# xiaozhah/Aligner

Hardware: AMD Instinct MI355X
Metric: aligned utterances/sec + frames/sec, [B=64,T_text=200,T_mel=1000] (higher is better)
Workload: dtype f32; 1 GPU; configs[1]: similarity (L2, C=80) + monotonic alignment search, [B=64,T_text=200,T_mel=1000] fp32 per GPU, dense fp32 path + int32 durations out; batch_per_gpu=64, t_text=200, t_mel=1000, c_att=80, launch=hipGraph, batches_in_flight=3, parallelism=batch-sharded x1

## Files before the change

aligner_amd/csrc/api.cpp:

```cpp
#include <cstdarg>
#include <cstdio>
#include <cstdlib>

#include <mutex>
#include <cstring>
#include <map>
#include <utility>

#include "common.h"

namespace aligner {

char *error_buffer() {
    static thread_local char buf[512] = {0};
    return buf;
}

unsigned long long *g_debug_stamps = nullptr;

static int env_flag(const char *name) { const char *e = getenv(name); return e && e[0] && e[0] != '0'; }
int g_opt_fwdsum_one_wave = env_flag("ALIGNER_FWDSUM_ONE_WAVE");
int g_opt_fwdsum_serial = env_flag("ALIGNER_FWDSUM_SERIAL");
int g_opt_fwdsum_no_grad_stager = 0;
int g_opt_softattn_exact = env_flag("ALIGNER_SOFTATTN_EXACT");
int g_opt_mobo_drop_segment = -1;
int g_opt_mobo_start_lag = 0;
int g_opt_mobo_lanes = 0;
int g_opt_mobo_bwd_general = 0;
int g_opt_softattn_no_pair = 0;
int g_opt_softattn_rt_drop_merge = 0;
int g_opt_softattn_strips = env_flag("ALIGNER_SOFTATTN_STRIPS");
int g_opt_softattn_split = 0;
int g_opt_conv_narrow_ft = 0;
int g_opt_conv_no_ring = 0;
int g_opt_conv_no_fuse = 0;
int g_opt_conv_split_always = env_flag("ALIGNER_CONV_SPLIT_ALWAYS");
int g_opt_maxpath_no_split_walk = 0;
int g_opt_maxpath_zero_blocks = 0;
int g_opt_maxpath_no_mask_verify = 0;
int g_opt_maxpath_no_optimistic_mask = 0;
int g_opt_mobo_full_chain = 0;
int g_opt_mobo_stamp_wave = 0;

hipError_t ensure_dynamic_lds(const void *kernel, size_t bytes) {
    if (bytes <= 64 * 1024) return hipSuccess;
    int dev = 0;
    hipError_t e = hipGetDevice(&dev);
    if (e != hipSuccess) return e;
    static std::mutex mu;
    static std::map<std::pair<int, const void *>, size_t> granted;
    std::lock_guard<std::mutex> lock(mu);
    const auto key = std::make_pair(dev, kernel);
    auto it = granted.find(key);
    if (it != granted.end() && it->second >= bytes) return hipSuccess;
    e = hipFuncSetAttribute(kernel, hipFuncAttributeMaxDynamicSharedMemorySize, (int)bytes);
    if (e == hipSuccess) granted[key] = bytes;
    return e;
}

int device_cu_count() {
    int dev = 0, v = 0;
    if (hipGetDevice(&dev) != hipSuccess) return 1;
    static std::mutex mu;
    static std::map<int, int> counts;
    std::lock_guard<std::mutex> lock(mu);
    auto it = counts.find(dev);
    if (it != counts.end()) return it->second;
    if (hipDeviceGetAttribute(&v, hipDeviceAttributeMultiprocessorCount, dev) != hipSuccess || v < 1) v = 1;
    counts[dev] = v;
    return v;
}

int device_lds_limit() {
    int dev = 0;
    if (hipGetDevice(&dev) != hipSuccess) return 64 * 1024;
    static std::mutex mu;
    static std::map<int, int> limits;
    std::lock_guard<std::mutex> lock(mu);
    auto it = limits.find(dev);
    if (it != limits.end()) return it->second;
    int lim = 64 * 1024, v = 0;
    hipDeviceProp_t prop;
    if (hipGetDeviceProperties(&prop, dev) == hipSuccess && std::strncmp(prop.gcnArchName, "gfx950", 6) == 0)
        lim = 160 * 1024;
    else if (hipDeviceGetAttribute(&v, hipDeviceAttributeMaxSharedMemoryPerBlock, dev) == hipSuccess && v > 0)
        lim = v;
    limits[dev] = lim;
    return lim;
}

int fail(int code, const char *fmt, ...) {
    va_list ap;
    va_start(ap, fmt);
    vsnprintf(error_buffer(), 512, fmt, ap);
    va_end(ap);
    return code;
}

}

extern "C" {

int aligner_abi_version(void) { return ALIGNER_ABI_VERSION; }

const char *aligner_last_error(void) { return aligner::error_buffer(); }

void aligner_debug_set_stamps(void *stamps_dev) {
    aligner::g_debug_stamps = static_cast<unsigned long long *>(stamps_dev);
}

int aligner_debug_set_option(const char *name, int value) {
    if (!name) return aligner::fail(ALIGNER_EINVAL, "null option name");
    if (std::strcmp(name, "fwdsum_one_wave") == 0) { aligner::g_opt_fwdsum_one_wave = value; return ALIGNER_OK; }
    if (std::strcmp(name, "fwdsum_no_grad_stager") == 0) { aligner::g_opt_fwdsum_no_grad_stager = value; return ALIGNER_OK; }
    if (std::strcmp(name, "fwdsum_serial") == 0) { aligner::g_opt_fwdsum_serial = value; return ALIGNER_OK; }
    if (std::strcmp(name, "softattn_exact") == 0) { aligner::g_opt_softattn_exact = value; return ALIGNER_OK; }
    if (std::strcmp(name, "mobo_start_lag") == 0) { aligner::g_opt_mobo_start_lag = value; return ALIGNER_OK; }
    if (std::strcmp(name, "mobo_lanes") == 0) { aligner::g_opt_mobo_lanes = value; return ALIGNER_OK; }
    if (std::strcmp(name, "mobo_stamp_wave") == 0) { aligner::g_opt_mobo_stamp_wave = value; return ALIGNER_OK; }
    if (std::strcmp(name, "mobo_full_chain") == 0) { aligner::g_opt_mobo_full_chain = value; return ALIGNER_OK; }
    if (std::strcmp(name, "softattn_split") == 0) { aligner::g_opt_softattn_split = value; return ALIGNER_OK; }
    if (std::strcmp(name, "conv_narrow_ft") == 0) { aligner::g_opt_conv_narrow_ft = value; return ALIGNER_OK; }
    if (std::strcmp(name, "conv_no_ring") == 0) { aligner::g_opt_conv_no_ring = value; return ALIGNER_OK; }
    if (std::strcmp(name, "conv_no_fuse") == 0) { aligner::g_opt_conv_no_fuse = value; return ALIGNER_OK; }
    if (std::strcmp(name, "conv_split_always") == 0) { aligner::g_opt_conv_split_always = value; return ALIGNER_OK; }
    if (std::strcmp(name, "maxpath_no_optimistic_mask") == 0) { aligner::g_opt_maxpath_no_optimistic_mask = value; return ALIGNER_OK; }
    if (std::strcmp(name, "maxpath_no_mask_verify") == 0) { aligner::g_opt_maxpath_no_mask_verify = value; return ALIGNER_OK; }
    if (std::strcmp(name, "maxpath_zero_blocks") == 0) { aligner::g_opt_maxpath_zero_blocks = value; return ALIGNER_OK; }
    if (std::strcmp(name, "maxpath_no_split_walk") == 0) { aligner::g_opt_maxpath_no_split_walk = value; return ALIGNER_OK; }
    if (std::strcmp(name, "softattn_strips") == 0) { aligner::g_opt_softattn_strips = value; return ALIGNER_OK; }
    if (std::strcmp(name, "softattn_rt_drop_merge") == 0) { aligner::g_opt_softattn_rt_drop_merge = value; return ALIGNER_OK; }
    if (std::strcmp(name, "softattn_no_pair") == 0) { aligner::g_opt_softattn_no_pair = value; return ALIGNER_OK; }
    if (std::strcmp(name, "mobo_bwd_general") == 0) { aligner::g_opt_mobo_bwd_general = value; return ALIGNER_OK; }
    if (std::strcmp(name, "mobo_drop_segment") == 0) { aligner::g_opt_mobo_drop_segment = value; return ALIGNER_OK; }
    return aligner::fail(ALIGNER_EINVAL, "unknown option '%s'", name);
}

int aligner_device_count(void) {
    int n = 0;
    if (hipGetDeviceCount(&n) != hipSuccess) {
        (void)hipGetLastError();
        return 0;
    }
    return n;
}

}
```

aligner_amd/csrc/common.h:

```cpp
#pragma once
#include <hip/hip_runtime.h>
#include <cstdarg>
#include <cstdio>

#include "aligner_amd.h"

namespace aligner {

char *error_buffer();
int   fail(int code, const char *fmt, ...) __attribute__((format(printf, 2, 3)));

#define ALIGNER_HIP_CHECK(expr)                                                        \
    do {                                                                               \
        hipError_t _e = (expr);                                                        \
        if (_e != hipSuccess)                                                          \
            return ::aligner::fail(ALIGNER_EHIP, "%s failed: %s (%s:%d)", #expr,       \
                                   hipGetErrorString(_e), __FILE__, __LINE__);         \
    } while (0)

inline int dtype_size(int dt) {
    switch (dt) {
        case ALIGNER_DT_F32: return 4;
        case ALIGNER_DT_F16: return 2;
        case ALIGNER_DT_BF16: return 2;
        case ALIGNER_DT_F64: return 8;
        case ALIGNER_DT_I32: return 4;
        case ALIGNER_DT_U8: return 1;
        case ALIGNER_DT_I64: return 8;
        default: return 0;
    }
}

hipError_t ensure_dynamic_lds(const void *kernel, size_t bytes);

int device_lds_limit();
int device_cu_count();

extern unsigned long long *g_debug_stamps;
extern int g_opt_softattn_exact;
extern int g_opt_mobo_start_lag;
extern int g_opt_mobo_stamp_wave;
extern int g_opt_mobo_full_chain;
extern int g_opt_conv_narrow_ft;
extern int g_opt_conv_no_ring;
extern int g_opt_maxpath_no_optimistic_mask;
extern int g_opt_maxpath_no_mask_verify;
extern int g_opt_maxpath_zero_blocks;
extern int g_opt_maxpath_no_split_walk;
extern int g_opt_conv_no_fuse;
extern int g_opt_conv_split_always;
extern int g_opt_softattn_split;
extern int g_opt_softattn_strips;
extern int g_opt_softattn_rt_drop_merge;
extern int g_opt_softattn_no_pair;
extern int g_opt_mobo_bwd_general;
extern int g_opt_mobo_lanes;
extern int g_opt_mobo_drop_segment;
extern int g_opt_fwdsum_no_grad_stager;
extern int g_opt_fwdsum_serial;
extern int g_opt_fwdsum_one_wave;

inline size_t align_up(size_t v, size_t a) { return (v + a - 1) / a * a; }

}
```

aligner_amd/csrc/mobo.hip:

```cpp
#include <hip/hip_runtime.h>

#include <cmath>
#include <cstdint>

#include "aligner_amd.h"
#include "common.h"

namespace aligner {

constexpr float MB_NEG = -1e30f;
constexpr float MB_DEADF = -1e7f;
constexpr int MB_DEADM = -(1 << 24);
constexpr unsigned MB_FILL = 0xFFFFFFFFu;
constexpr float MB_LOG2E = 1.4426950408889634f, MB_LN2 = 0.6931471805599453f;
constexpr int MB_SPIN_LIMIT = 1 << 21;

struct MoboParams {
    const void *e;
    const int *t_xs, *t_ys;
    float *log_alpha;
    int *boundaries;
    int *durations;
    float *map_score;
    float *Lw;
// ... 225 lines not shown
    __syncthreads();
    const int Rb = s_blockmax;
    bool fits = true;
    for (int x = tid; x < NE; x += 256) {
        const int M = sM[x];
        sT[x] = __builtin_ldexpf(sS[x], M - Rb);
        if (M != MB_DEADM && M < Rb - 100) fits = false;
    }
    const int slow = __syncthreads_or(!fits);
    const int xb = 4 * tid;
    float Ls[4] = {MB_NEG, MB_NEG, MB_NEG, MB_NEG};
    if (k0 + xb < p.Ty) {
        if (!slow && D >= 8) {
            const float *t = sT + xb;
            const float4 h = *reinterpret_cast<const float4 *>(t);
            float core = h.w;
            int c = 4;
            for (; c + 8 <= D; c += 8) {
                const float4 a = *reinterpret_cast<const float4 *>(t + c), bq = *reinterpret_cast<const float4 *>(t + c + 4);
                core += ((a.x + a.y) + (a.z + a.w)) + ((bq.x + bq.y) + (bq.z + bq.w));
            }
            for (; c < D; ++c) core += t[c];
            const float e0 = t[D], e1 = t[D + 1], e2 = t[D + 2];
            const float acc[4] = {core + ((h.x + h.y) + h.z), core + ((h.y + h.z) + e0), core + ((h.z + e0) + e1),
                                  core + ((e0 + e1) + e2)};
#pragma unroll
            for (int u = 0; u < 4; ++u)
                if (acc[u] > 0.f) Ls[u] = (float)Rb + __builtin_amdgcn_logf(acc[u]);
        } else if (!slow) {
#pragma unroll 1
            for (int u = 0; u < 4; ++u) {
                float acc = 0.f;
                for (int c = 0; c < D; ++c) acc += sT[xb + u + c];
                if (acc > 0.f) Ls[u] = (float)Rb + __builtin_amdgcn_logf(acc);
            }
        } else {
#pragma unroll 1
            for (int u = 0; u < 4; ++u) {
                int Mw, qb;
                float acc, best;
                mb_window<false>(sM + xb + u, sS + xb + u, nullptr, D, Mw, acc, best, qb);
                if (acc > 0.f) Ls[u] = (float)Mw + __builtin_amdgcn_logf(acc);
            }
        }
#pragma unroll
        for (int u = 0; u < 4; ++u) {
            const int k = k0 + xb + u;
            if (k < p.Ty) {
                p.Lw[rowoff + k] = (k < J && k >= klo && k <= khi) ? Ls[u] : MB_NEG;
                if (p.log_alpha && k >= J) p.log_alpha[rowoff + k] = -__builtin_huge_valf();
            }
        }
    }
}

__device__ __forceinline__ void mb_ring_store(unsigned *p, unsigned v) {
    __hip_atomic_store(p, v, __ATOMIC_RELAXED, __HIP_MEMORY_SCOPE_AGENT);
}
__device__ __forceinline__ unsigned mb_ring_load(const unsigned *p) {
    return __hip_atomic_load(p, __ATOMIC_RELAXED, __HIP_MEMORY_SCOPE_AGENT);
}

struct MbSeg {
    int a, bnd, D, J, W;
    bool has_next;
    int *sM;
    float *sS, *sV;
    unsigned *ring_out;
};
__device__ __forceinline__ void mb_phase1(const MbSeg &g, int i, int bo, int k, float la, float de, float Lraw) {
    const float L = (k < g.J) ? Lraw : MB_NEG;
    const bool live = L > MB_DEADF;
    const float u = (live && la > MB_DEADF) ? la - L : MB_NEG;
    float v = (live && de > MB_DEADF) ? de - L : MB_NEG;
    v = (v > MB_DEADF) ? v : MB_NEG;
    int M;
    float s;
    mb_encode(u, M, s);
    const int x = bo + g.D + (k - g.a);
    g.sM[x] = M;
    g.sS[x] = s;
    g.sV[x] = v;
    if (g.has_next && k >= g.bnd - g.D) {
        unsigned *r = g.ring_out + (size_t)i * 3 * g.D + (k - (g.bnd - g.D));
        mb_ring_store(r, __builtin_bit_cast(unsigned, (float)M));
        mb_ring_store(r + g.D, __builtin_bit_cast(unsigned, s));
        mb_ring_store(r + 2 * g.D, __builtin_bit_cast(unsigned, v));
    }
}
__device__ __forceinline__ void mb_phase2(const MbSeg &g, int bo, int j, int lo, int hi, float ev, float &lav, float &dev,
                                          int &dur) {
    lav = MB_NEG;
    dev = MB_NEG;
    dur = 0;
    if (j >= lo && j <= hi) {
        int Mw, qb;
        float acc, best;
        const int x = bo + (j - g.a);
        mb_window<true>(g.sM + x, g.sS + x, g.sV + x, g.D, Mw, acc, best, qb);
        if (acc > 0.f && ev > MB_DEADF) lav = ev + ((float)Mw + __builtin_amdgcn_logf(acc));
        if (best > MB_DEADF && ev > MB_DEADF) {
            dev = ev + best;
            dur = g.D - qb;
        }
        lav = (lav > MB_DEADF) ? lav : MB_NEG;
        dev = (dev > MB_DEADF) ? dev : MB_NEG;
// ... 967 lines not shown
                for (const int r8 = cnt & 7; c < r8; ++c) acc += t[c];
                for (; c < cnt; c += 8)
                    acc += ((t[c] + t[c + 1]) + (t[c + 2] + t[c + 3])) + ((t[c + 4] + t[c + 5]) + (t[c + 6] + t[c + 7]));
#pragma unroll
                for (int m = 1; m < H; m <<= 1) acc += mb_quad_xor_f(acc, m);
                if (acc > 0.f) lsum = (float)R + __builtin_amdgcn_logf(acc);
            } else {
                int Mw, qb;
                float acc, best;
                mb_window<false>(sM + x, sS + x, nullptr, cnt, Mw, acc, best, qb);
#pragma unroll
                for (int m = 1; m < H; m <<= 1) {
                    const int Mo = mb_quad_xor_i(Mw, m);
                    const float ao = mb_quad_xor_f(acc, m);
                    const int Mn = Mw > Mo ? Mw : Mo;
                    acc = __builtin_ldexpf(acc, Mw - Mn) + __builtin_ldexpf(ao, Mo - Mn);
                    Mw = Mn;
                }
                if (acc > 0.f) lsum = (float)Mw + __builtin_amdgcn_logf(acc);
            }
            float lav = MB_NEG;
            if (feasible && ev > MB_DEADF && lsum > MB_DEADF) lav = ev + lsum;
            lav = (lav > MB_DEADF) ? lav : MB_NEG;
            la = lav;
            R = (Rn != MB_DEADM) ? Rn : R;
            float *lp = (lead && j1 >= 1) ? p.log_alpha + ro + (j1 - 1) : reinterpret_cast<float *>(trash);
            *lp = (lav > MB_DEADF) ? lav * MB_LN2 : -__builtin_huge_valf();
        }
    };
#pragma unroll 1
    for (int i = i0; i <= i1; i += 2) {
        do_row(i, e_n1, L_n1);
        if (i + 1 > i1) break;
        do_row(i + 1, e_n2, L_n2);
    }
    if (i1 + 1 < I) {
        const int i = i1 + 1;
        if (publishes) {
            const float Lr = p.Lw[ubase + (size_t)i * p.Ty + kl];
            const float L = (j1 < J) ? Lr : MB_NEG;
            const float u = (L > MB_DEADF && la > MB_DEADF) ? la - L : MB_NEG;
            int M;
            float sm;
            mb_encode(u, M, sm);
            unsigned *r = ring_out + (size_t)i * 3 * D + (j1 - (bnd - D));
            mb_ring_store(r, __builtin_bit_cast(unsigned, (float)M));
            mb_ring_store(r + D, __builtin_bit_cast(unsigned, sm));
        }
        if (lead && j1 >= 1) p.log_alpha[ubase + (size_t)i * p.Ty + (j1 - 1)] = -__builtin_huge_valf();
        dead_rows(i1 + 2, I);
    }
}

__global__ __launch_bounds__(256) void mobo_backtrack_kernel(MoboParams p, int RB) {
    extern __shared__ __attribute__((aligned(16))) unsigned char smem[];
    __shared__ int s_j, s_bad;
    __shared__ int s_b[64], s_d[64];
    typedef unsigned piece_t __attribute__((ext_vector_type(4)));
    piece_t *win = reinterpret_cast<piece_t *>(smem);
    const int tid = threadIdx.x, b = blockIdx.x, D = p.D;
    int I = p.t_xs[b], J = p.t_ys[b];
    I = I > p.Tx ? p.Tx : I;
    J = J > p.Ty ? p.Ty : J;
    const bool ok = I >= 1 && J >= I && (long long)J <= (long long)I * D;
    int *bo = p.boundaries + (size_t)b * p.Tx;
    int *du = p.durations ? p.durations + (size_t)b * p.Tx : nullptr;
    if (!ok || p.failw[b]) {
        for (int i = tid; i < p.Tx; i += 256) {
            bo[i] = 0;
            if (du) du[i] = 0;
        }
        if (p.map_score && tid == 0) p.map_score[b] = -__builtin_huge_valf();
        return;
    }
    for (int i = I + tid; i < p.Tx; i += 256) {
        bo[i] = J;
        if (du) du[i] = 0;
    }
    const unsigned short *backb = p.back + (size_t)b * p.Tx * p.bstride;
    const int tpr = 256 / RB, t_of = tid / tpr, c_of = tid - t_of * tpr;
    const int wp = ((RB - 1) * D + 8) / 8 + 1;
    if (tid == 0) { s_j = J; s_bad = 0; }
    __syncthreads();
    for (int i = I - 1; i >= 0; i -= RB) {
        const int nb = (i + 1 < RB) ? i + 1 : RB;
        const int j = s_j;
        {
            const int t = t_of;
            int first = j - t * D;
            first = first < 0 ? 0 : first;
            const int p0 = first >> 3, p1 = (j - t) >> 3;
            const piece_t *src = reinterpret_cast<const piece_t *>(backb + (size_t)(i - t) * p.bstride);
            piece_t r[16];
#pragma unroll
            for (int q = 0; q < 16; ++q) {
                const int pc = p0 + c_of + q * tpr;
                r[q] = (t < nb && j >= t && pc <= p1) ? __builtin_nontemporal_load(src + pc) : piece_t{0, 0, 0, 0};
            }
#pragma unroll
            for (int q = 0; q < 16; ++q) {
                const int pc = c_of + q * tpr;
                if (pc < wp) win[t * wp + pc] = r[q];
            }
        }
        __syncthreads();
        if (tid == 0) {
            const unsigned short *w16 = reinterpret_cast<const unsigned short *>(win);
            int jj = j;
            for (int t = 0; t < nb; ++t) {
                int first = j - t * D;
                first = first < 0 ? 0 : first;
                const int d = w16[(size_t)t * wp * 8 + (jj - (first & ~7))];
                s_b[t] = jj;
                s_d[t] = d;
                if (d < 1 || d > D || d > jj) { s_bad = (i == I - 1 && t == 0 && d == 0) ? 2 : 1; jj = 0; break; }
                jj -= d;
            }
            s_j = jj;
        }
        __syncthreads();
        if (s_bad) break;
        if (tid < nb) {
            bo[i - tid] = s_b[tid];
            if (du) du[i - tid] = s_d[tid];
        }
        __syncthreads();
    }
    if (s_bad) {
        for (int i = tid; i < p.Tx; i += 256) {
            bo[i] = 0;
            if (du) du[i] = 0;
        }
        if (p.map_score && tid == 0) p.map_score[b] = -__builtin_huge_valf();
        if (tid == 0) atomicOr(p.status, s_bad == 2 ? ALIGNER_ST_BAD_LENGTHS : ALIGNER_ST_INTERNAL);
    } else if (tid == 0 && s_j != 0) {
        atomicOr(p.status, ALIGNER_ST_INTERNAL);
    }
}

__global__ __launch_bounds__(256) void mobo_gamma_kernel(const float *__restrict__ log_alpha, const int *__restrict__ t_xs,
                                                          const int *__restrict__ t_ys, float *__restrict__ gamma,
                                                          int Tx, int Ty) {
    __shared__ float wsum[2][4];
    __shared__ float carry[2];
    const int i = blockIdx.x, b = blockIdx.y, tid = threadIdx.x, lane = tid & 63, wave = tid >> 6;
    int I = t_xs[b], J = t_ys[b];
    I = I > Tx ? Tx : I;
    J = J > Ty ? Ty : J;
    float *g = gamma + ((size_t)b * Tx + i) * Ty;
    if (i >= I || I < 1 || J < I) {
        for (int y = tid; y < Ty; y += 256) g[y] = 0.f;
        return;
    }
    const float *cur = log_alpha + ((size_t)b * Tx + i) * Ty;
    const float *prv = cur - Ty;
    if (tid == 0) { carry[0] = 0.f; carry[1] = 0.f; }
    __syncthreads();
    for (int y0 = 0; y0 < Ty; y0 += 256) {
        const int y = y0 + tid;
        float a0 = (y < J) ? __expf(cur[y]) : 0.f;
        float a1 = (i > 0 && y < J) ? __expf(prv[y]) : 0.f;
        float s0 = a0, s1 = a1;
#pragma unroll
        for (int off = 1; off < 64; off <<= 1) {
            const float t0 = __shfl_up(s0, off), t1 = __shfl_up(s1, off);
            if (lane >= off) { s0 += t0; s1 += t1; }
        }
        if (lane == 63) { wsum[0][wave] = s0; wsum[1][wave] = s1; }
        __syncthreads();
        float base0 = carry[0], base1 = carry[1];
        for (int w = 0; w < wave; ++w) { base0 += wsum[0][w]; base1 += wsum[1][w]; }
        const float c0 = base0 + s0 - a0, c1 = base1 + s1 - a1;
        if (y < Ty) g[y] = (y < J) ? ((i > 0 ? c1 : 1.f) - c0) : 0.f;
        __syncthreads();
        if (tid == 255) { carry[0] = base0 + s0; carry[1] = base1 + s1; }
        __syncthreads();
    }
}

#include "mobo_bwd.inc"

struct MoboPlan {
    int D, S, nmax, NP, T, RB, bstride, H;
    size_t lds, bt_lds, ring_words;
    size_t status_off, fail_off, trash_off, L_off, back_off, ring_off, total;
};

static int mobo_plan(int B, int Tx, int Ty, int max_duration, MoboPlan &pl, bool quiet) {
    const int D = max_duration > Ty ? Ty : max_duration;
    const int P = Ty + 1;
    const int cu = device_cu_count();
    const int lds_limit = device_lds_limit();
    const int smax = P / D < 1 ? 1 : P / D;
    int S = cu / (B < 1 ? 1 : B);
    S = S < 1 ? 1 : S;
    S = S > smax ? smax : S;
    const int swave = (P + 63) / 64;
    S = S > swave ? swave : S;
    int nmax = 0;
    size_t lds = 0;
    for (;; ++S) {
        const int n1 = (P + S - 1) / S, n2 = (2 * D < P) ? 2 * D : P;
        nmax = n1 > n2 ? n1 : n2;
        lds = nmax > 1024 ? (size_t)2 * 3 * 4 * ((size_t)nmax + D) + (size_t)8 * nmax
                          : (size_t)2 * 4 * 4 * ((size_t)nmax + D) + 64 * sizeof(int);
        if (lds <= (size_t)lds_limit) break;
        if (S >= smax)
            return quiet ? ALIGNER_EDOM
                         : fail(ALIGNER_EDOM, "Ty=%d with max_duration=%d needs %zu bytes of LDS per segment (limit %d)", Ty,
                                D, lds, lds_limit);
    }
    pl.D = D;
    pl.S = S;
    pl.nmax = nmax;
    pl.NP = nmax <= 1024 ? 1 : 2;
    pl.H = nmax <= 64 ? 4 : nmax <= 128 ? 2 : 1;
    if (g_opt_mobo_lanes == 1 || g_opt_mobo_lanes == 2 || g_opt_mobo_lanes == 4)
        if ((long long)nmax * g_opt_mobo_lanes <= 1024) pl.H = g_opt_mobo_lanes;
    pl.T = nmax <= 1024 ? (nmax * pl.H + 63) / 64 * 64 : 1024;
    if (nmax <= 1024 && S > 1) {
        if (pl.T + 64 > 1024) { pl.H = 1; pl.T = (nmax + 63) / 64 * 64; }
        if (pl.T + 64 <= 1024) pl.T += 64;
        else pl.NP = 2;
    }
    pl.lds = lds;
    int RB = 32;
    while (RB > 1 && (long long)RB * RB * D > 32768) RB >>= 1;
    pl.RB = RB;
    pl.bt_lds = (size_t)RB * (((size_t)(RB - 1) * D + 8) / 8 + 1) * 16;
    pl.ring_words = (size_t)B * (S - 1) * Tx * 3 * D;
    pl.status_off = 0;
    pl.fail_off = 256;
    pl.trash_off = align_up(pl.fail_off + (size_t)B * sizeof(int), 256);
    pl.L_off = align_up(pl.trash_off + ((size_t)B * S * 1024 + 64) * sizeof(unsigned), 256);
    pl.back_off = align_up(pl.L_off + (size_t)B * Tx * Ty * sizeof(float), 256);
    pl.bstride = (Ty + 1 + 7) / 8 * 8;
    pl.ring_off = align_up(pl.back_off + (size_t)B * Tx * pl.bstride * sizeof(unsigned short), 256);
    pl.total = align_up(pl.ring_off + pl.ring_words * sizeof(unsigned), 256);
    return ALIGNER_OK;
}

struct MoboBwdPlan {
    MoboPlan f;
    int T;
    bool multi;
    size_t lds, ring_words;
    size_t status_off, fail_off, trash_off, L_off, G_off, Y_off, ring_off, total;
};
static int mobo_bwd_plan(int B, int Tx, int Ty, int max_duration, MoboBwdPlan &pl, bool quiet) {
    const int rc = mobo_plan(B, Tx, Ty, max_duration, pl.f, quiet);
    if (rc) return rc;
    const MoboPlan &f = pl.f;
    pl.multi = f.NP != 1;
    pl.T = f.T;
    pl.lds = f.lds;
    pl.ring_words = (size_t)B * (f.S - 1) * Tx * 2 * f.D;
    const size_t cells = align_up((size_t)B * Tx * Ty * sizeof(float), 256);
    pl.status_off = 0;
    pl.fail_off = 256;
    pl.trash_off = align_up(pl.fail_off + (size_t)B * sizeof(int), 256);
    pl.L_off = align_up(pl.trash_off + ((size_t)B * f.S * 1024 + 64) * sizeof(unsigned), 256);
    pl.G_off = pl.L_off + cells;
    pl.Y_off = pl.G_off + cells;
    pl.ring_off = pl.Y_off + cells;
    pl.total = align_up(pl.ring_off + pl.ring_words * sizeof(unsigned), 256);
    return ALIGNER_OK;
}

}

using namespace aligner;

extern "C" {

size_t aligner_boundary_search_backward_workspace_bytes(int B, int Tx, int Ty, int max_duration) {
    if (B < 0 || Tx < 1 || Ty < 1 || max_duration < 1) return 0;
    MoboBwdPlan pl;
    if (mobo_bwd_plan(B, Tx, Ty, max_duration, pl, true) != ALIGNER_OK) return 0;
    return pl.total;
}

int aligner_boundary_search_backward(const void *energies, int energy_dtype, const int32_t *t_xs, const int32_t *t_ys,
                                     int max_duration, const float *log_alpha, const float *grad_log_alpha,
                                     const float *grad_gamma, float *grad_energies_out, void *workspace,
                                     size_t workspace_bytes, int B, int Tx, int Ty, void *stream) {
    if (!energies || !t_xs || !t_ys || !log_alpha || !grad_energies_out || !workspace) return fail(ALIGNER_EINVAL, "null pointer");
    if (!grad_log_alpha && !grad_gamma) return fail(ALIGNER_EINVAL, "no cotangent: grad_log_alpha and grad_gamma are both null");
    if (B < 0 || Tx < 1 || Ty < 1) return fail(ALIGNER_EINVAL, "bad shape B=%d Tx=%d Ty=%d", B, Tx, Ty);
    if (max_duration < 1) return fail(ALIGNER_EINVAL, "max_duration %d < 1", max_duration);
    const int vt = energy_dtype == ALIGNER_DT_F32 ? 0 : energy_dtype == ALIGNER_DT_BF16 ? 1 : energy_dtype == ALIGNER_DT_F16 ? 2 : -1;
    if (vt < 0) return fail(ALIGNER_EINVAL, "energy dtype %d not supported (F32, BF16, F16)", energy_dtype);
    if (B == 0) return ALIGNER_OK;
    if (B > 65535 || Tx > 65535) return fail(ALIGNER_EDOM, "grid too large");
    if ((max_duration > Ty ? Ty : max_duration) > 65535) return fail(ALIGNER_EDOM, "max_duration %d too large", max_duration);
    MoboBwdPlan pl;
    const int prc = mobo_bwd_plan(B, Tx, Ty, max_duration, pl, false);
    if (prc) return prc;
    const MoboPlan &f = pl.f;
    if ((long long)B * f.S > 0x7fffffffLL) return fail(ALIGNER_EDOM, "grid too large");
    if (workspace_bytes < pl.total) return fail(ALIGNER_ENOSPC, "workspace %zu < %zu bytes", workspace_bytes, pl.total);
    unsigned char *ws = static_cast<unsigned char *>(workspace);
    hipStream_t s = static_cast<hipStream_t>(stream);
    const size_t nlds = (size_t)(MB_NCH + f.D + 4) * 12;
    if (nlds > (size_t)device_lds_limit()) return fail(ALIGNER_EDOM, "max_duration %d needs %zu bytes of LDS", f.D, nlds);
    {
        MoboParams p{};
        p.e = energies;  p.t_xs = t_xs;  p.t_ys = t_ys;
        p.Lw = reinterpret_cast<float *>(ws + pl.L_off);
        p.ring = reinterpret_cast<unsigned *>(ws + pl.ring_off);
        p.failw = reinterpret_cast<int *>(ws + pl.fail_off);
        p.status = reinterpret_cast<int *>(ws + pl.status_off);
        p.B = B;  p.Tx = Tx;  p.Ty = Ty;  p.D = f.D;  p.S = f.S;  p.nmax = f.nmax;
        const dim3 grid((Ty + MB_NCH - 1) / MB_NCH, Tx, B);
        auto launch = [&](auto kern) -> int {
            ALIGNER_HIP_CHECK(ensure_dynamic_lds(reinterpret_cast<const void *>(kern), nlds));
            hipLaunchKernelGGL(kern, grid, dim3(256), nlds, s, p, (unsigned long long)pl.ring_words);
            ALIGNER_HIP_CHECK(hipGetLastError());
            return ALIGNER_OK;
        };
        const int rc = vt == 0 ? launch(mobo_norm_kernel<0>) : vt == 1 ? launch(mobo_norm_kernel<1>) : launch(mobo_norm_kernel<2>);
        if (rc) return rc;
    }
    float *Gw = reinterpret_cast<float *>(ws + pl.G_off);
    MoboBwdParams q{energies, t_xs, t_ys, log_alpha, grad_log_alpha, grad_gamma, grad_energies_out,
                    reinterpret_cast<float *>(ws + pl.L_off), grad_gamma ? Gw : grad_log_alpha, Gw,
                    reinterpret_cast<float *>(ws + pl.Y_off), reinterpret_cast<unsigned *>(ws + pl.ring_off),
                    reinterpret_cast<int *>(ws + pl.fail_off), reinterpret_cast<unsigned *>(ws + pl.trash_off),
                    reinterpret_cast<int *>(ws + pl.status_off), B, Tx, Ty, f.D, f.S, f.nmax, g_opt_mobo_start_lag,
                    g_opt_mobo_drop_segment, g_opt_mobo_drop_segment >= 0 ? 2048 : MB_SPIN_LIMIT, g_debug_stamps, g_opt_mobo_stamp_wave};
    if (grad_gamma) {
        hipLaunchKernelGGL(mobo_bwd_cotangent_kernel, dim3(Tx, B), dim3(256), 0, s, q);
        ALIGNER_HIP_CHECK(hipGetLastError());
    }
    {
        auto launch = [&](auto kern) -> int {
            ALIGNER_HIP_CHECK(ensure_dynamic_lds(reinterpret_cast<const void *>(kern), pl.lds));
            hipLaunchKernelGGL(kern, dim3((unsigned)B * f.S), dim3(pl.T), pl.lds, s, q);
            ALIGNER_HIP_CHECK(hipGetLastError());
            return ALIGNER_OK;
        };
#define MB_BWD_LAUNCH(VT_)                                                                                             \
    (pl.multi ? launch(mobo_bwd_chain_kernel<VT_, true>)                                                              \
     : g_opt_mobo_bwd_general ? launch(mobo_bwd_chain_kernel<VT_, false>)                                             \
     : g_debug_stamps ? MB_BWD_LAUNCH_H(VT_, true) : MB_BWD_LAUNCH_H(VT_, false))
#define MB_BWD_LAUNCH_H(VT_, ST_)                                                                                     \
    (f.H == 1 ? launch(mobo_bwd_chain_one_kernel<VT_, 1, ST_>) : f.H == 2 ? launch(mobo_bwd_chain_one_kernel<VT_, 2, ST_>) \
                                                                           : launch(mobo_bwd_chain_one_kernel<VT_, 4, ST_>))
        if (g_opt_mobo_bwd_general && !pl.multi) pl.T = (f.nmax + 63) / 64 * 64;
        const int rc = vt == 0 ? MB_BWD_LAUNCH(0) : vt == 1 ? MB_BWD_LAUNCH(1) : MB_BWD_LAUNCH(2);
#undef MB_BWD_LAUNCH
#undef MB_BWD_LAUNCH_H
        if (rc) return rc;
    }
    {
        const dim3 grid((Ty + MB_NCH - 1) / MB_NCH, Tx, B);
        auto launch = [&](auto kern) -> int {
            ALIGNER_HIP_CHECK(ensure_dynamic_lds(reinterpret_cast<const void *>(kern), nlds));
            hipLaunchKernelGGL(kern, grid, dim3(256), nlds, s, q);
            ALIGNER_HIP_CHECK(hipGetLastError());
            return ALIGNER_OK;
        };
        const int rc = vt == 0 ? launch(mobo_bwd_grad_kernel<0>) : vt == 1 ? launch(mobo_bwd_grad_kernel<1>) : launch(mobo_bwd_grad_kernel<2>);
        if (rc) return rc;
    }
    return ALIGNER_OK;
}

size_t aligner_boundary_search_workspace_bytes_ex(int B, int Tx, int Ty, int max_duration) {
    if (B < 0 || Tx < 1 || Ty < 1 || max_duration < 1) return 0;
    MoboPlan pl;
    if (mobo_plan(B, Tx, Ty, max_duration, pl, true) != ALIGNER_OK) return 0;
    return pl.total;
}

size_t aligner_boundary_search_workspace_bytes(int B, int Tx, int Ty) {
    if (B < 0 || Tx < 1 || Ty < 1) return 0;
    const size_t fixed = 256 + align_up((size_t)B * sizeof(int), 256) + align_up((size_t)B * Tx * Ty * sizeof(float), 256) +
                         align_up(((size_t)(B > 1024 ? B : 1024 + B) * 1024 + 64) * sizeof(unsigned), 256) +
                         align_up((size_t)B * Tx * ((size_t)Ty + 8) * sizeof(unsigned short), 256);
    return fixed + align_up((size_t)B * Tx * 3 * ((size_t)Ty + 1) * sizeof(unsigned), 256) + 256;
}

int aligner_boundary_search(const void *energies, int energy_dtype, const int32_t *t_xs, const int32_t *t_ys,
                            int max_duration, int32_t *boundaries_out, int32_t *durations_out, float *map_score_out,
                            float *log_alpha_out, float *gamma_out, void *workspace, size_t workspace_bytes, int B,
                            int Tx, int Ty, void *stream) {
    if (!energies || !t_xs || !t_ys || !workspace) return fail(ALIGNER_EINVAL, "null pointer");
    if (!boundaries_out && !log_alpha_out) return fail(ALIGNER_EINVAL, "nothing asked for: boundaries_out and log_alpha_out are both null");
    if (!boundaries_out && (durations_out || map_score_out))
        return fail(ALIGNER_EINVAL, "durations / map_score need boundaries_out (the MAP sequence is searched or it is not)");
    if (B < 0 || Tx < 1 || Ty < 1) return fail(ALIGNER_EINVAL, "bad shape B=%d Tx=%d Ty=%d", B, Tx, Ty);
    if (max_duration < 1) return fail(ALIGNER_EINVAL, "max_duration %d < 1", max_duration);
    const int vt = energy_dtype == ALIGNER_DT_F32 ? 0 : energy_dtype == ALIGNER_DT_BF16 ? 1 : energy_dtype == ALIGNER_DT_F16 ? 2 : -1;
    if (vt < 0) return fail(ALIGNER_EINVAL, "energy dtype %d not supported (F32, BF16, F16)", energy_dtype);
    if (gamma_out && !log_alpha_out) return fail(ALIGNER_EINVAL, "gamma needs the log_alpha buffer as well");
    if (B == 0) return ALIGNER_OK;
    if (B > 65535 || Tx > 65535) return fail(ALIGNER_EDOM, "grid too large");
    if ((max_duration > Ty ? Ty : max_duration) > 65535) return fail(ALIGNER_EDOM, "max_duration %d too large", max_duration);
    MoboPlan pl;
    const int prc = mobo_plan(B, Tx, Ty, max_duration, pl, false);
    if (prc) return prc;
    if ((long long)B * pl.S > 0x7fffffffLL) return fail(ALIGNER_EDOM, "grid too large");
    if (workspace_bytes < pl.total) return fail(ALIGNER_ENOSPC, "workspace %zu < %zu bytes", workspace_bytes, pl.total);
    unsigned char *ws = static_cast<unsigned char *>(workspace);
    hipStream_t s = static_cast<hipStream_t>(stream);
    MoboParams p{energies, t_xs, t_ys, log_alpha_out, boundaries_out, durations_out, map_score_out,
                 reinterpret_cast<float *>(ws + pl.L_off), reinterpret_cast<unsigned short *>(ws + pl.back_off),
                 reinterpret_cast<unsigned *>(ws + pl.ring_off), reinterpret_cast<int *>(ws + pl.fail_off),
                 reinterpret_cast<unsigned *>(ws + pl.trash_off),
                 reinterpret_cast<int *>(ws + pl.status_off), B, Tx, Ty, pl.D, pl.S, pl.nmax, pl.bstride, g_opt_mobo_start_lag, g_debug_stamps,
                 g_opt_mobo_drop_segment, g_opt_mobo_drop_segment >= 0 ? 2048 : MB_SPIN_LIMIT};
    {
        const size_t nlds = (size_t)(MB_NCH + pl.D + 4) * 12;
        if (nlds > (size_t)device_lds_limit()) return fail(ALIGNER_EDOM, "max_duration %d needs %zu bytes of LDS", pl.D, nlds);
        const dim3 grid((Ty + MB_NCH - 1) / MB_NCH, Tx, B);
        auto launch = [&](auto kern) -> int {
            ALIGNER_HIP_CHECK(ensure_dynamic_lds(reinterpret_cast<const void *>(kern), nlds));
            hipLaunchKernelGGL(kern, grid, dim3(256), nlds, s, p, (unsigned long long)pl.ring_words);
            ALIGNER_HIP_CHECK(hipGetLastError());
            return ALIGNER_OK;
        };
        const int rc = vt == 0 ? launch(mobo_norm_kernel<0>) : vt == 1 ? launch(mobo_norm_kernel<1>) : launch(mobo_norm_kernel<2>);
        if (rc) return rc;
    }
    {
        auto launch = [&](auto kern) -> int {
            ALIGNER_HIP_CHECK(ensure_dynamic_lds(reinterpret_cast<const void *>(kern), pl.lds));
            hipLaunchKernelGGL(kern, dim3((unsigned)B * pl.S), dim3(pl.T), pl.lds, s, p);
            ALIGNER_HIP_CHECK(hipGetLastError());
            return ALIGNER_OK;
        };
        int rc;
#define MB_LAUNCH_NP(VT_)                                                                               \
    (pl.NP != 1 ? launch(mobo_chain_kernel<VT_, true>)                                                  \
     : (!boundaries_out && !g_opt_mobo_full_chain && !g_debug_stamps) ? MB_LAUNCH_SUM(VT_)              \
     : log_alpha_out ? MB_LAUNCH_H(VT_, true)                                                           \
     : (g_opt_mobo_full_chain || g_debug_stamps) ? MB_LAUNCH_H(VT_, false) : MB_LAUNCH_MAP(VT_))
#define MB_LAUNCH_SUM(VT_)                                                                              \
    (pl.H == 1 ? launch(mobo_chain_sum_kernel<VT_, 1>) : pl.H == 2 ? launch(mobo_chain_sum_kernel<VT_, 2>) \
                                                                    : launch(mobo_chain_sum_kernel<VT_, 4>))
#define MB_LAUNCH_MAP(VT_)                                                                              \
    (pl.H == 1 ? launch(mobo_chain_map_kernel<VT_, 1>) : pl.H == 2 ? launch(mobo_chain_map_kernel<VT_, 2>) \
                                                                    : launch(mobo_chain_map_kernel<VT_, 4>))
#define MB_LAUNCH_H(VT_, LA_)                                                                            \
    (g_debug_stamps ? MB_LAUNCH_ST(VT_, LA_, true) : MB_LAUNCH_ST(VT_, LA_, false))
#define MB_LAUNCH_ST(VT_, LA_, ST_)                                                                      \
    (pl.H == 1 ? launch(mobo_chain_one_kernel<VT_, LA_, 1, ST_>) : pl.H == 2 ? launch(mobo_chain_one_kernel<VT_, LA_, 2, ST_>) \
                                                                              : launch(mobo_chain_one_kernel<VT_, LA_, 4, ST_>))
        rc = vt == 0 ? MB_LAUNCH_NP(0) : vt == 1 ? MB_LAUNCH_NP(1) : MB_LAUNCH_NP(2);
        if (rc) return rc;
    }
    if (boundaries_out) {
        ALIGNER_HIP_CHECK(ensure_dynamic_lds(reinterpret_cast<const void *>(mobo_backtrack_kernel), pl.bt_lds));
        hipLaunchKernelGGL(mobo_backtrack_kernel, dim3(B), dim3(256), pl.bt_lds, s, p, pl.RB);
        ALIGNER_HIP_CHECK(hipGetLastError());
    }
    if (gamma_out) {
        hipLaunchKernelGGL(mobo_gamma_kernel, dim3(Tx, B), dim3(256), 0, s, log_alpha_out, t_xs, t_ys, gamma_out, Tx, Ty);
        ALIGNER_HIP_CHECK(hipGetLastError());
    }
    return ALIGNER_OK;
}

}
```

Before: 2.135 million utterances/s.

## Add streaming log-norm kernel and double-buffered prefetching backtrack for MoBo

Replaces the MoBo normalization kernel with a streaming variant. It loads quads with vector loads, finds a block-wide max exponent, and sums scaled window terms in LDS, falling back to the exact window path only when the dynamic range is too wide. It also adds a backtrack kernel that double-buffers the back-pointer window in LDS and prefetches the next row block into registers while one wavefront walks the current block with readlane. This is meant to hide global-load latency in the serial backtrack and cut norm cost, at the price of extra registers and LDS plus more complex bounds logic.

Measured after the change: 2.103 million utterances/s. -1.5%, worse.

```diff
diff --git a/aligner_amd/csrc/api.cpp b/aligner_amd/csrc/api.cpp
--- a/aligner_amd/csrc/api.cpp
+++ b/aligner_amd/csrc/api.cpp
@@ -41,6 +41,8 @@
 int g_opt_maxpath_no_optimistic_mask = 0;
 int g_opt_mobo_full_chain = 0;
 int g_opt_mobo_stamp_wave = 0;
+int g_opt_mobo_backtrack_v1 = 0;
+int g_opt_mobo_norm_v1 = 0;
 
 hipError_t ensure_dynamic_lds(const void *kernel, size_t bytes) {
     if (bytes <= 64 * 1024) return hipSuccess;
@@ -133,6 +135,8 @@
     if (std::strcmp(name, "softattn_no_pair") == 0) { aligner::g_opt_softattn_no_pair = value; return ALIGNER_OK; }
     if (std::strcmp(name, "mobo_bwd_general") == 0) { aligner::g_opt_mobo_bwd_general = value; return ALIGNER_OK; }
     if (std::strcmp(name, "mobo_drop_segment") == 0) { aligner::g_opt_mobo_drop_segment = value; return ALIGNER_OK; }
+    if (std::strcmp(name, "mobo_backtrack_v1") == 0) { aligner::g_opt_mobo_backtrack_v1 = value; return ALIGNER_OK; }
+    if (std::strcmp(name, "mobo_norm_v1") == 0) { aligner::g_opt_mobo_norm_v1 = value; return ALIGNER_OK; }
     return aligner::fail(ALIGNER_EINVAL, "unknown option '%s'", name);
 }
 
diff --git a/aligner_amd/csrc/common.h b/aligner_amd/csrc/common.h
--- a/aligner_amd/csrc/common.h
+++ b/aligner_amd/csrc/common.h
@@ -56,6 +56,8 @@
 extern int g_opt_mobo_bwd_general;
 extern int g_opt_mobo_lanes;
 extern int g_opt_mobo_drop_segment;
+extern int g_opt_mobo_backtrack_v1;
+extern int g_opt_mobo_norm_v1;
 extern int g_opt_fwdsum_no_grad_stager;
 extern int g_opt_fwdsum_serial;
 extern int g_opt_fwdsum_one_wave;
diff --git a/aligner_amd/csrc/mobo.hip b/aligner_amd/csrc/mobo.hip
--- a/aligner_amd/csrc/mobo.hip
+++ b/aligner_amd/csrc/mobo.hip
@@ -301,6 +301,209 @@
             }
         }
     }
+}
+
+template <int VT> __device__ __forceinline__ void mb_load_quad(const void *base, size_t idx, bool wide, int n, unsigned (&raw)[4]) {
+    if (wide) {
+        if (VT == 0) {
+            const uint4 q = *reinterpret_cast<const uint4 *>(static_cast<const unsigned *>(base) + idx);
+            raw[0] = q.x;  raw[1] = q.y;  raw[2] = q.z;  raw[3] = q.w;
+        } else {
+            const uint2 q = *reinterpret_cast<const uint2 *>(static_cast<const unsigned short *>(base) + idx);
+            raw[0] = q.x & 0xFFFFu;  raw[1] = q.x >> 16;  raw[2] = q.y & 0xFFFFu;  raw[3] = q.y >> 16;
+        }
+    } else {
+#pragma unroll
+        for (int u = 0; u < 4; ++u) raw[u] = mb_load_raw<VT>(base, idx + (u < n ? u : n - 1));
+    }
+}
+
+template <int VT>
+__global__ __launch_bounds__(256) void mobo_lnorm_stream_kernel(MoboParams p, unsigned long long ring_words) {
+    extern __shared__ __attribute__((aligned(16))) unsigned char smem[];
+    __shared__ int s_wavemax[4];
+    const int tid = threadIdx.x;
+    const int b = blockIdx.z, i = blockIdx.y, k0 = blockIdx.x * MB_NCH;
+    {
+        const unsigned long long nthr = (unsigned long long)gridDim.x * gridDim.y * gridDim.z * 256ull;
+        const unsigned long long gid = (((unsigned long long)b * gridDim.y + i) * gridDim.x + blockIdx.x) * 256ull + tid;
+        for (unsigned long long w = gid; w < ring_words; w += nthr) p.ring[w] = MB_FILL;
+        if (gid < (unsigned long long)p.B) p.failw[gid] = 0;
+    }
+    const int D = p.D;
+    int I = p.t_xs[b], J = p.t_ys[b];
+    I = I > p.Tx ? p.Tx : I;
+    J = J > p.Ty ? p.Ty : J;
+    const bool ok = I >= 1 && J >= I && (long long)J <= (long long)I * D;
+    const size_t rowoff = ((size_t)b * p.Tx + i) * p.Ty;
+    const int xb = 4 * tid, kq = k0 + xb;
+    const int nq = p.Ty - kq < 4 ? p.Ty - kq : 4;
+    if (!ok || i >= I) {
+        if (p.log_alpha)
+            for (int u = 0; u < nq; ++u) p.log_alpha[rowoff + kq + u] = -__builtin_huge_valf();
+        return;
+    }
+    const bool quads = (p.Ty & 3) == 0;
+    const bool wide_st = quads && (reinterpret_cast<uintptr_t>(p.Lw) & 15) == 0;
+    auto store_L = [&](const float (&L)[4]) {
+        if (nq <= 0) return;
+        if (wide_st) {
+            *reinterpret_cast<float4 *>(p.Lw + rowoff + kq) = float4{L[0], L[1], L[2], L[3]};
+        } else {
+#pragma unroll
+            for (int u = 0; u < 4; ++u)
+                if (u < nq) p.Lw[rowoff + kq + u] = L[u];
+        }
+        if (p.log_alpha) {
+#pragma unroll
+            for (int u = 0; u < 4; ++u)
+                if (u < nq && kq + u >= J) p.log_alpha[rowoff + kq + u] = -__builtin_huge_valf();
+        }
+    };
+    int lo, hi;
+    mb_bounds(I, J, D, i, lo, hi);
+    int klo = 0, khi = 0;
+    if (i > 0) {
+        mb_bounds(I, J, D, i - 1, klo, khi);
+        const long long reach = (long long)i * D;
+        if (khi > reach) khi = (int)reach;
+    }
+    if (k0 > khi || k0 + MB_NCH - 1 < klo) {
+        const float dead[4] = {MB_NEG, MB_NEG, MB_NEG, MB_NEG};
+        store_L(dead);
+        return;
+    }
+    const int NE = MB_NCH + D;
+    const int NEp = (NE + 3) & ~3;
+    int *sM = reinterpret_cast<int *>(smem);
+    float *sS = reinterpret_cast<float *>(sM + NEp);
+    float *sT = sS + NEp;
+    const bool wide_ld = quads && (reinterpret_cast<uintptr_t>(p.e) & (VT == 0 ? 15 : 7)) == 0;
+    unsigned raw[4] = {0, 0, 0, 0}, rawh = 0;
+    if (nq > 0) mb_load_quad<VT>(p.e, rowoff + kq, wide_ld, nq, raw);
+    const int xh = MB_NCH + tid;
+    {
+        int f = k0 + xh;
+        f = f < p.Ty ? f : p.Ty - 1;
+        if (xh < NE) rawh = mb_load_raw<VT>(p.e, rowoff + f);
+    }
+    auto entry = [&](unsigned r, int x, int &M, float &s) {
+        const int m = k0 + 1 + x;
+        mb_encode((m >= lo && m <= hi) ? mb_value<VT>(r) * MB_LOG2E : MB_NEG, M, s);
+    };
+    auto far_entry = [&](int x, int &M, float &s) {
+        const int m = k0 + 1 + x;
+        const unsigned r = (m >= lo && m <= hi) ? mb_load_raw<VT>(p.e, rowoff + (m - 1)) : 0u;
+        entry(r, x, M, s);
+    };
+    int Mq[4], Mh = MB_DEADM, Mmax = MB_DEADM;
+    float sq[4], sh = 0.f;
+#pragma unroll
+    for (int u = 0; u < 4; ++u) {
+        entry(raw[u], xb + u, Mq[u], sq[u]);
+        Mmax = Mmax > Mq[u] ? Mmax : Mq[u];
+    }
+    if (xh < NE) {
+        entry(rawh, xh, Mh, sh);
+        Mmax = Mmax > Mh ? Mmax : Mh;
+    }
+    for (int x = xh + 256; x < NE; x += 256) {
+        int M;
+        float s;
+        far_entry(x, M, s);
+        Mmax = Mmax > M ? Mmax : M;
+    }
+    {
+        const int wm = mb_wave_max_i32(Mmax);
+        if ((tid & 63) == 0) s_wavemax[tid >> 6] = wm;
+    }
+    __syncthreads();
+    int Rb = s_wavemax[0];
+#pragma unroll
+    for (int w = 1; w < 4; ++w) Rb = Rb > s_wavemax[w] ? Rb : s_wavemax[w];
+    bool fits = true;
+    {
+        float4 t4;
+        t4.x = __builtin_ldexpf(sq[0], Mq[0] - Rb);
+        t4.y = __builtin_ldexpf(sq[1], Mq[1] - Rb);
+        t4.z = __builtin_ldexpf(sq[2], Mq[2] - Rb);
+        t4.w = __builtin_ldexpf(sq[3], Mq[3] - Rb);
+        *reinterpret_cast<float4 *>(sT + xb) = t4;
+#pragma unroll
+        for (int u = 0; u < 4; ++u)
+            if (Mq[u] != MB_DEADM && Mq[u] < Rb - 100) fits = false;
+        if (xh < NE) {
+            sT[xh] = __builtin_ldexpf(sh, Mh - Rb);
+            if (Mh != MB_DEADM && Mh < Rb - 100) fits = false;
+        }
+        for (int x = xh + 256; x < NE; x += 256) {
+            int M;
+            float s;
+            far_entry(x, M, s);
+            sT[x] = __builtin_ldexpf(s, M - Rb);
+            if (M != MB_DEADM && M < Rb - 100) fits = false;
+        }
+    }
+    const int slow = __syncthreads_or(!fits);
+    if (slow) {
+#pragma unroll
+        for (int u = 0; u < 4; ++u) {
+            sM[xb + u] = Mq[u];
+            sS[xb + u] = sq[u];
+        }
+        if (xh < NE) {
+            sM[xh] = Mh;
+            sS[xh] = sh;
+        }
+        for (int x = xh + 256; x < NE; x += 256) {
+            int M;
+            float s;
+            far_entry(x, M, s);
+            sM[x] = M;
+            sS[x] = s;
+        }
+        __syncthreads();
+    }
+    if (nq <= 0) return;
+    float Ls[4] = {MB_NEG, MB_NEG, MB_NEG, MB_NEG};
+    if (!slow && D >= 8) {
+        const float *t = sT + xb;
+        const float4 h = *reinterpret_cast<const float4 *>(t);
+        float core = h.w;
+        int c = 4;
+        for (; c + 8 <= D; c += 8) {
+            const float4 a = *reinterpret_cast<const float4 *>(t + c), bq = *reinterpret_cast<const float4 *>(t + c + 4);
+            core += ((a.x + a.y) + (a.z + a.w)) + ((bq.x + bq.y) + (bq.z + bq.w));
+        }
+        for (; c < D; ++c) core += t[c];
+        const float e0 = t[D], e1 = t[D + 1], e2 = t[D + 2];
+        const float acc[4] = {core + ((h.x + h.y) + h.z), core + ((h.y + h.z) + e0), core + ((h.z + e0) + e1),
+                              core + ((e0 + e1) + e2)};
+#pragma unroll
+        for (int u = 0; u < 4; ++u)
+            if (acc[u] > 0.f) Ls[u] = (float)Rb + __builtin_amdgcn_logf(acc[u]);
+    } else if (!slow) {
+#pragma unroll
+        for (int u = 0; u < 4; ++u) {
+            float acc = 0.f;
+            for (int c = 0; c < D; ++c) acc += sT[xb + u + c];
+            if (acc > 0.f) Ls[u] = (float)Rb + __builtin_amdgcn_logf(acc);
+        }
+    } else {
+#pragma unroll
+        for (int u = 0; u < 4; ++u) {
+            int Mw, qb;
+            float acc, best;
+            mb_window<false>(sM + xb + u, sS + xb + u, nullptr, D, Mw, acc, best, qb);
+            if (acc > 0.f) Ls[u] = (float)Mw + __builtin_amdgcn_logf(acc);
+        }
+    }
+#pragma unroll
+    for (int u = 0; u < 4; ++u) {
+        const int k = kq + u;
+        Ls[u] = (k < J && k >= klo && k <= khi) ? Ls[u] : MB_NEG;
+    }
+    store_L(Ls);
 }
 
 __device__ __forceinline__ void mb_ring_store(unsigned *p, unsigned v) {
@@ -1374,9 +1577,15 @@
     }
 }
 
+constexpr int MB_BT_STAMP_ROW = 3072;
+
+template <bool STAMPS>
 __global__ __launch_bounds__(256) void mobo_backtrack_kernel(MoboParams p, int RB) {
     extern __shared__ __attribute__((aligned(16))) unsigned char smem[];
     __shared__ int s_j, s_bad;
+    const bool stamping = STAMPS && p.stamps != nullptr && threadIdx.x == 0;
+    unsigned long long st_t = 0, st_acc[3] = {0, 0, 0}, st_n = 0;
+#define MB_BT_STAMP(k_) if (stamping) { const unsigned long long t_ = __builtin_amdgcn_s_memrealtime(); st_acc[k_] += t_ - st_t; st_t = t_; }
     __shared__ int s_b[64], s_d[64];
     typedef unsigned piece_t __attribute__((ext_vector_type(4)));
     piece_t *win = reinterpret_cast<piece_t *>(smem);
@@ -1404,9 +1613,11 @@
     const int wp = ((RB - 1) * D + 8) / 8 + 1;
     if (tid == 0) { s_j = J; s_bad = 0; }
     __syncthreads();
+    if (stamping) st_t = __builtin_amdgcn_s_memrealtime();
     for (int i = I - 1; i >= 0; i -= RB) {
         const int nb = (i + 1 < RB) ? i + 1 : RB;
         const int j = s_j;
+        if (stamping) ++st_n;
         {
             const int t = t_of;
             int first = j - t * D;
@@ -1426,6 +1637,7 @@
             }
         }
         __syncthreads();
+        MB_BT_STAMP(0)
         if (tid == 0) {
             const unsigned short *w16 = reinterpret_cast<const unsigned short *>(win);
             int jj = j;
@@ -1440,6 +1652,7 @@
             }
             s_j = jj;
         }
+        MB_BT_STAMP(1)
         __syncthreads();
         if (s_bad) break;
         if (tid < nb) {
@@ -1447,6 +1660,12 @@
             if (du) du[i - tid] = s_d[tid];
         }
         __syncthreads();
+        MB_BT_STAMP(2)
+    }
+#undef MB_BT_STAMP
+    if (stamping) {
+        unsigned long long *o = p.stamps + (size_t)(MB_BT_STAMP_ROW + b) * 24;
+        o[0] = st_acc[0];  o[1] = st_acc[1];  o[2] = st_acc[2];  o[3] = st_n;  o[4] = (unsigned long long)RB;
     }
     if (s_bad) {
         for (int i = tid; i < p.Tx; i += 256) {
@@ -1456,6 +1675,125 @@
         if (p.map_score && tid == 0) p.map_score[b] = -__builtin_huge_valf();
         if (tid == 0) atomicOr(p.status, s_bad == 2 ? ALIGNER_ST_BAD_LENGTHS : ALIGNER_ST_INTERNAL);
     } else if (tid == 0 && s_j != 0) {
+        atomicOr(p.status, ALIGNER_ST_INTERNAL);
+    }
+}
+
+constexpr int MB_BT_NQ = 10;
+
+template <bool STAMPS>
+__global__ __launch_bounds__(256) void mobo_backtrack_ahead_kernel(MoboParams p, int RB, int wp) {
+    extern __shared__ __attribute__((aligned(16))) unsigned char smem[];
+    __shared__ int s_end[2];
+    typedef unsigned piece_t __attribute__((ext_vector_type(4)));
+    piece_t *win = reinterpret_cast<piece_t *>(smem);
+    const int tid = threadIdx.x, b = blockIdx.x, D = p.D;
+    const bool stamping = STAMPS && p.stamps != nullptr && tid == 0;
+    unsigned long long st_t = 0, st_acc[3] = {0, 0, 0}, st_n = 0;
+#define MB_BT_STAMP(k_) if (stamping) { const unsigned long long t_ = __builtin_amdgcn_s_memrealtime(); st_acc[k_] += t_ - st_t; st_t = t_; }
+    int I = p.t_xs[b], J = p.t_ys[b];
+    I = I > p.Tx ? p.Tx : I;
+    J = J > p.Ty ? p.Ty : J;
+    const bool ok = I >= 1 && J >= I && (long long)J <= (long long)I * D;
+    int *bo = p.boundaries + (size_t)b * p.Tx;
+    int *du = p.durations ? p.durations + (size_t)b * p.Tx : nullptr;
+    if (!ok || p.failw[b]) {
+        for (int i = tid; i < p.Tx; i += 256) {
+            bo[i] = 0;
+            if (du) du[i] = 0;
+        }
+        if (p.map_score && tid == 0) p.map_score[b] = -__builtin_huge_valf();
+        return;
+    }
+    for (int i = I + tid; i < p.Tx; i += 256) {
+        bo[i] = J;
+        if (du) du[i] = 0;
+    }
+    const unsigned short *backb = p.back + (size_t)b * p.Tx * p.bstride;
+    const int tpr = 256 / RB, t_of = tid / tpr, c_of = tid - t_of * tpr;
+    piece_t r[MB_BT_NQ];
+    auto issue = [&](int top, int jb, int k0) {
+        const int tok = top - t_of, k = k0 + t_of;
+        int first = jb - k * D;
+        first = first < 0 ? 0 : first;
+        const int last = jb - k;
+        const int p0 = first >> 3, p1 = last >> 3;
+        const piece_t *src = reinterpret_cast<const piece_t *>(backb + (size_t)(tok < 0 ? 0 : tok) * p.bstride);
+#pragma unroll
+        for (int q = 0; q < MB_BT_NQ; ++q) {
+            const int pc = p0 + c_of + q * tpr;
+            r[q] = (tok >= 0 && last >= 0 && pc <= p1) ? __builtin_nontemporal_load(src + pc) : piece_t{0, 0, 0, 0};
+        }
+    };
+    auto land = [&](int buf) {
+        piece_t *dst = win + (size_t)(buf * RB + t_of) * wp;
+#pragma unroll
+        for (int q = 0; q < MB_BT_NQ; ++q) {
+            const int pc = c_of + q * tpr;
+            if (pc < wp) dst[pc] = r[q];
+        }
+    };
+    issue(I - 1, J, 0);
+    land(0);
+    __syncthreads();
+    if (stamping) st_t = __builtin_amdgcn_s_memrealtime();
+    int j = J, jb = J, k0 = 0, bad = 0;
+    for (int top = I - 1, n = 0; top >= 0; top -= RB, ++n) {
+        const int nb = (top + 1 < RB) ? top + 1 : RB;
+        const int cur = n & 1;
+        const bool more = top - RB >= 0;
+        if (stamping) ++st_n;
+        if (more) issue(top - RB, j, RB);
+        MB_BT_STAMP(0)
+        int mypos = 0, mydur = 0;
+        if (tid < 64) {
+            const unsigned short *w16 = reinterpret_cast<const unsigned short *>(win);
+            int off = 0;
+            if (tid < RB) {
+                int first = jb - (k0 + tid) * D;
+                first = first < 0 ? 0 : first;
+                off = (cur * RB + tid) * wp * 8 - (first & ~7);
+            }
+            int jj = __builtin_amdgcn_readfirstlane(j), wbad = 0;
+            for (int t = 0; t < nb; ++t) {
+                const int o = __builtin_amdgcn_readlane(off, t);
+                const int d = __builtin_amdgcn_readfirstlane((int)w16[o + jj]);
+                if (tid == t) {
+                    mypos = jj;
+                    mydur = d;
+                }
+                if (d < 1 || d > D || d > jj) { wbad = (top == I - 1 && t == 0 && d == 0) ? 2 : 1; break; }
+                jj -= d;
+            }
+            if (tid == 0) s_end[cur] = wbad ? -wbad : jj;
+        }
+        MB_BT_STAMP(1)
+        if (more) land(cur ^ 1);
+        __syncthreads();
+        const int v = s_end[cur];
+        if (v < 0) { bad = -v; break; }
+        if (tid < nb) {
+            bo[top - tid] = mypos;
+            if (du) du[top - tid] = mydur;
+        }
+        jb = j;
+        k0 = RB;
+        j = v;
+        MB_BT_STAMP(2)
+    }
+#undef MB_BT_STAMP
+    if (stamping) {
+        unsigned long long *o = p.stamps + (size_t)(MB_BT_STAMP_ROW + b) * 24;
+        o[0] = st_acc[0];  o[1] = st_acc[1];  o[2] = st_acc[2];  o[3] = st_n;  o[4] = (unsigned long long)RB;
+    }
+    if (bad) {
+        for (int i = tid; i < p.Tx; i += 256) {
+            bo[i] = 0;
+            if (du) du[i] = 0;
+        }
+        if (p.map_score && tid == 0) p.map_score[b] = -__builtin_huge_valf();
+        if (tid == 0) atomicOr(p.status, bad == 2 ? ALIGNER_ST_BAD_LENGTHS : ALIGNER_ST_INTERNAL);
+    } else if (tid == 0 && j != 0) {
         atomicOr(p.status, ALIGNER_ST_INTERNAL);
     }
 }
@@ -1504,7 +1842,8 @@
 
 struct MoboPlan {
     int D, S, nmax, NP, T, RB, bstride, H;
-    size_t lds, bt_lds, ring_words;
+    int RB2, wp2;
+    size_t lds, bt_lds, bt_lds2, ring_words;
     size_t status_off, fail_off, trash_off, L_off, back_off, ring_off, total;
 };
 
@@ -1550,6 +1889,19 @@
     while (RB > 1 && (long long)RB * RB * D > 32768) RB >>= 1;
     pl.RB = RB;
     pl.bt_lds = (size_t)RB * (((size_t)(RB - 1) * D + 8) / 8 + 1) * 16;
+    pl.RB2 = 0;
+    pl.wp2 = 0;
+    pl.bt_lds2 = 0;
+    for (int r2 = 32; r2 >= 1; r2 >>= 1) {
+        const size_t wp2 = ((size_t)(2 * r2 - 1) * (D - 1)) / 8 + 2;
+        const size_t tpr2 = 256 / r2;
+        if (2 * r2 * wp2 * 16 <= 64 * 1024 && (wp2 + tpr2 - 1) / tpr2 <= (size_t)MB_BT_NQ) {
+            pl.RB2 = r2;
+            pl.wp2 = (int)wp2;
+            pl.bt_lds2 = 2 * r2 * wp2 * 16;
+            break;
+        }
+    }
     pl.ring_words = (size_t)B * (S - 1) * Tx * 3 * D;
     pl.status_off = 0;
     pl.fail_off = 256;
@@ -1640,7 +1992,11 @@
             ALIGNER_HIP_CHECK(hipGetLastError());
             return ALIGNER_OK;
         };
-        const int rc = vt == 0 ? launch(mobo_norm_kernel<0>) : vt == 1 ? launch(mobo_norm_kernel<1>) : launch(mobo_norm_kernel<2>);
+        const int rc = g_opt_mobo_norm_v1
+                           ? (vt == 0 ? launch(mobo_norm_kernel<0>) : vt == 1 ? launch(mobo_norm_kernel<1>) : launch(mobo_norm_kernel<2>))
+                           : (vt == 0   ? launch(mobo_lnorm_stream_kernel<0>)
+                              : vt == 1 ? launch(mobo_lnorm_stream_kernel<1>)
+                                        : launch(mobo_lnorm_stream_kernel<2>));
         if (rc) return rc;
     }
     float *Gw = reinterpret_cast<float *>(ws + pl.G_off);
@@ -1742,7 +2098,11 @@
             ALIGNER_HIP_CHECK(hipGetLastError());
             return ALIGNER_OK;
         };
-        const int rc = vt == 0 ? launch(mobo_norm_kernel<0>) : vt == 1 ? launch(mobo_norm_kernel<1>) : launch(mobo_norm_kernel<2>);
+        const int rc = g_opt_mobo_norm_v1
+                           ? (vt == 0 ? launch(mobo_norm_kernel<0>) : vt == 1 ? launch(mobo_norm_kernel<1>) : launch(mobo_norm_kernel<2>))
+                           : (vt == 0   ? launch(mobo_lnorm_stream_kernel<0>)
+                              : vt == 1 ? launch(mobo_lnorm_stream_kernel<1>)
+                                        : launch(mobo_lnorm_stream_kernel<2>));
         if (rc) return rc;
     }
     {
@@ -1773,9 +2133,18 @@
         if (rc) return rc;
     }
     if (boundaries_out) {
-        ALIGNER_HIP_CHECK(ensure_dynamic_lds(reinterpret_cast<const void *>(mobo_backtrack_kernel), pl.bt_lds));
-        hipLaunchKernelGGL(mobo_backtrack_kernel, dim3(B), dim3(256), pl.bt_lds, s, p, pl.RB);
-        ALIGNER_HIP_CHECK(hipGetLastError());
+        const bool ahead = pl.RB2 > 0 && !g_opt_mobo_backtrack_v1;
+        auto launch = [&](auto kern, size_t lds, auto... extra) -> int {
+            ALIGNER_HIP_CHECK(ensure_dynamic_lds(reinterpret_cast<const void *>(kern), lds));
+            hipLaunchKernelGGL(kern, dim3(B), dim3(256), lds, s, p, extra...);
+            ALIGNER_HIP_CHECK(hipGetLastError());
+            return ALIGNER_OK;
+        };
+        const int rc = ahead ? (g_debug_stamps ? launch(mobo_backtrack_ahead_kernel<true>, pl.bt_lds2, pl.RB2, pl.wp2)
+                                               : launch(mobo_backtrack_ahead_kernel<false>, pl.bt_lds2, pl.RB2, pl.wp2))
+                             : (g_debug_stamps ? launch(mobo_backtrack_kernel<true>, pl.bt_lds, pl.RB)
+                                               : launch(mobo_backtrack_kernel<false>, pl.bt_lds, pl.RB));
+        if (rc) return rc;
     }
     if (gamma_out) {
         hipLaunchKernelGGL(mobo_gamma_kernel, dim3(Tx, B), dim3(256), 0, s, log_alpha_out, t_xs, t_ys, gamma_out, Tx, Ty);
```
